# BatsResearch/menghini-neurips23-code

Hardware: AMD Instinct MI355X
Metric: images/sec CLIP ViT-B/16 encode+prompt-step (higher is better)
Workload: dtype f16

## Files before the change

### menghini-neurips23-code_amd/csrc/attention_split.hip

```cpp
#include <math.h>

#include "common.h"

__device__ __forceinline__ int vt_index_fwd_s(int key, int d) { return vt_index(key, ((d >> 2) & 3) * 16 + (d >> 4) * 4 + (d & 3)); }

__device__ __forceinline__ void split8(const f32x4 a, const f32x4 b, half8& hi, half8& lo) {
    half4 h0, l0, h1, l1;
    split_f16x4(a, h0, l0);
    split_f16x4(b, h1, l1);
    hi = (half8){h0[0], h0[1], h0[2], h0[3], h1[0], h1[1], h1[2], h1[3]};
    lo = (half8){l0[0], l0[1], l0[2], l0[3], l1[0], l1[1], l1[2], l1[3]};
}

template <int KVC, bool CAUSAL, int NW>
__global__ __launch_bounds__(NW * 64) void attn_fwd_split_kernel(const float* __restrict__ qkv, half_t* __restrict__ out, int S, int H) {
    constexpr int SP = KVC * 32;
    constexpr float LOG2E = 1.4426950408889634f;
    constexpr float INV = 1.0f / (float)GRIP_SPLIT_LO_SCALE;
    extern __shared__ __attribute__((aligned(16))) char smem[];
    half_t* Kh = (half_t*)smem;
    half_t* Kl = Kh + SP * 64;
    half_t* Vh = Kl + SP * 64;
    half_t* Vl = Vh + SP * 64;

    const int tid = threadIdx.x, lane = tid & 63, wave = tid >> 6;
    const int D = H * 64;
    const int b = blockIdx.x / H, h = blockIdx.x - b * H;
    const size_t ld = (size_t)3 * D;
    const float* base = qkv + (size_t)b * S * ld + h * 64;
    const int li = lane & 15, lg = lane >> 4;
    const int n_qt = (S + 15) >> 4;

    for (int idx = tid; idx < SP * 8; idx += NW * 64) {
        const int row = idx >> 3, chunk = idx & 7;
        f32x4 a = {0.f, 0.f, 0.f, 0.f}, c = {0.f, 0.f, 0.f, 0.f};
        if (row < S) {
            const f32x4* p = (const f32x4*)(base + (size_t)row * ld + D + chunk * 8);
            a = p[0];
            c = p[1];
        }
        half8 hi, lo;
        split8(a, c, hi, lo);
        const int o = row * 64 + ((chunk ^ (row & 7)) * 8);
        *(half8*)(Kh + o) = hi;
        *(half8*)(Kl + o) = lo;
    }
    for (int idx = tid; idx < ((SP / 2 + 31) / 32) * 256; idx += NW * 64) {
        const int lane_rp = idx & 31, chunk = ((idx >> 5) & 1) + 2 * ((idx >> 6) & 3), rblk = idx >> 8;
        const int r0 = 2 * (rblk * 32 + lane_rp);
        if (r0 >= SP) continue;
        f32x4 z = {0.f, 0.f, 0.f, 0.f};
        f32x4 a0 = z, a1 = z, b0 = z, b1 = z;
        if (r0 < S) { const f32x4* p = (const f32x4*)(base + (size_t)r0 * ld + 2 * D + chunk * 8); a0 = p[0]; a1 = p[1]; }
        if (r0 + 1 < S) { const f32x4* p = (const f32x4*)(base + (size_t)(r0 + 1) * ld + 2 * D + chunk * 8); b0 = p[0]; b1 = p[1]; }
        half8 h0, l0, h1, l1;
        split8(a0, a1, h0, l0);
        split8(b0, b1, h1, l1);
#pragma unroll
        for (int j = 0; j < 8; ++j) {
            const int o = vt_index_fwd_s(r0, chunk * 8 + j);
            *(half2v*)(Vh + o) = (half2v){h0[j], h1[j]};
            *(half2v*)(Vl + o) = (half2v){l0[j], l1[j]};
        }
    }
    __syncthreads();

    for (int qt = wave; qt < n_qt; qt += NW) {
        asm volatile("" ::: "memory");
        const int qrow = qt * 16 + li;
        const int qr = qrow < S ? qrow : S - 1;
        half8 qh[2], ql[2];
#pragma unroll
        for (int kk = 0; kk < 2; ++kk) {
            const f32x4* p = (const f32x4*)(base + (size_t)qr * ld + (kk * 4 + lg) * 8);
            split8(p[0] * 0.125f, p[1] * 0.125f, qh[kk], ql[kk]);
        }
        f32x4 sc[2 * KVC];
        float m = -INFINITY;
#pragma unroll
        for (int t = 0; t < 2 * KVC; ++t) {
            f32x4 acc = {0.f, 0.f, 0.f, 0.f}, cor = {0.f, 0.f, 0.f, 0.f};
#pragma unroll
            for (int kk = 0; kk < 2; ++kk) {
                const int o = (t * 16 + li) * 64 + (((kk * 4 + lg) ^ (lane & 7)) * 8);
                const half8 kh = *(const half8*)(Kh + o), kl = *(const half8*)(Kl + o);
                acc = __builtin_amdgcn_mfma_f32_16x16x32_f16(kh, qh[kk], acc, 0, 0, 0);
                cor = __builtin_amdgcn_mfma_f32_16x16x32_f16(kl, qh[kk], cor, 0, 0, 0);
                cor = __builtin_amdgcn_mfma_f32_16x16x32_f16(kh, ql[kk], cor, 0, 0, 0);
            }
            acc += cor * INV;
            if (CAUSAL || t >= 2 * (KVC - 1)) {
#pragma unroll
                for (int r = 0; r < 4; ++r) {
                    const int kv = t * 16 + lg * 4 + r;
                    if (kv >= S || (CAUSAL && kv > qrow)) acc[r] = -INFINITY;
                }
            }
            m = fmaxf(fmaxf(fmaxf(m, acc[0]), fmaxf(acc[1], acc[2])), acc[3]);
            sc[t] = acc;
        }
        m = fmaxf(m, __shfl_xor(m, 16));
        m = fmaxf(m, __shfl_xor(m, 32));
        const float m2 = m * LOG2E;
#pragma unroll
        for (int t = 0; t < 2 * KVC; ++t)
#pragma unroll
            for (int r = 0; r < 4; ++r) sc[t][r] = __builtin_amdgcn_exp2f(__builtin_fmaf(sc[t][r], LOG2E, -m2));

        const half8 ones = {1, 1, 1, 1, 1, 1, 1, 1};
        f32x4 sum_h = {0.f, 0.f, 0.f, 0.f}, sum_l = {0.f, 0.f, 0.f, 0.f};
        f32x4 o[4], oc[4];
#pragma unroll
        for (int nf = 0; nf < 4; ++nf) { o[nf] = (f32x4){0.f, 0.f, 0.f, 0.f}; oc[nf] = (f32x4){0.f, 0.f, 0.f, 0.f}; }
#pragma unroll
        for (int c = 0; c < KVC; ++c) {
            half8 ph, pl;
            split8(sc[2 * c], sc[2 * c + 1], ph, pl);
#pragma unroll
            for (int nf = 0; nf < 4; ++nf) {
                const int vo = (c * 4 + nf) * 512 + (lg * 16 + (li ^ lg)) * 8;
                const half8 vh = *(const half8*)(Vh + vo), vl = *(const half8*)(Vl + vo);
                o[nf] = __builtin_amdgcn_mfma_f32_16x16x32_f16(vh, ph, o[nf], 0, 0, 0);
                oc[nf] = __builtin_amdgcn_mfma_f32_16x16x32_f16(vl, ph, oc[nf], 0, 0, 0);
                oc[nf] = __builtin_amdgcn_mfma_f32_16x16x32_f16(vh, pl, oc[nf], 0, 0, 0);
            }
            sum_h = __builtin_amdgcn_mfma_f32_16x16x32_f16(ones, ph, sum_h, 0, 0, 0);
            sum_l = __builtin_amdgcn_mfma_f32_16x16x32_f16(ones, pl, sum_l, 0, 0, 0);
        }
        if (qrow < S) {
            const float inv = 1.0f / (sum_h[0] + sum_l[0] * INV);
            half_t* orow = out + (size_t)((size_t)b * S + qrow) * 2 * D;
            const int col = h * 64 + lg * 16;
            half_t* op = orow + (col >> 5) * 64 + (col & 31);
            half8 hi0, lo0, hi1, lo1;
            split8((o[0] + oc[0] * INV) * inv, (o[1] + oc[1] * INV) * inv, hi0, lo0);
            split8((o[2] + oc[2] * INV) * inv, (o[3] + oc[3] * INV) * inv, hi1, lo1);
            *(half8*)op = hi0;
            *(half8*)(op + 8) = hi1;
            *(half8*)(op + 32) = lo0;
            *(half8*)(op + 40) = lo1;
        }
    }
}

bool attention_split_supported(int S) { return S >= 1 && S <= 320; }

int launch_attention_fwd_split(const float* qkv, void* out, int B, int S, int H, int causal, hipStream_t s) {
    GRIP_REQUIRE(attention_split_supported(S) && B >= 1 && H >= 1, "attention_split: bad shape B=%d S=%d H=%d (S <= 320)", B, S, H);
    const int kvc = (S + 31) / 32;
    const size_t lds = (size_t)4 * kvc * 32 * 64 * sizeof(half_t);
#define GRIP_ATT_CASE(K)                                                                                                                     \
    case K: {                                                                                                                                \
        static bool configured = false;                                                                                                      \
        if (!configured) {                                                                                                                   \
            GRIP_CHECK_HIP(hipFuncSetAttribute((const void*)attn_fwd_split_kernel<K, false, (K >= 4 ? 8 : 4)>, hipFuncAttributeMaxDynamicSharedMemorySize, (int)lds)); \
            GRIP_CHECK_HIP(hipFuncSetAttribute((const void*)attn_fwd_split_kernel<K, true, (K >= 4 ? 8 : 4)>, hipFuncAttributeMaxDynamicSharedMemorySize, (int)lds));  \
            configured = true;                                                                                                               \
        }                                                                                                                                    \
        if (causal) hipLaunchKernelGGL((attn_fwd_split_kernel<K, true, (K >= 4 ? 8 : 4)>), dim3(B * H), dim3((K >= 4 ? 8 : 4) * 64), lds, s, qkv, (half_t*)out, S, H); \
        else hipLaunchKernelGGL((attn_fwd_split_kernel<K, false, (K >= 4 ? 8 : 4)>), dim3(B * H), dim3((K >= 4 ? 8 : 4) * 64), lds, s, qkv, (half_t*)out, S, H);       \
    } break;
    switch (kvc) {
        GRIP_ATT_CASE(1) GRIP_ATT_CASE(2) GRIP_ATT_CASE(3) GRIP_ATT_CASE(4) GRIP_ATT_CASE(5)
        GRIP_ATT_CASE(6) GRIP_ATT_CASE(7) GRIP_ATT_CASE(8) GRIP_ATT_CASE(9) GRIP_ATT_CASE(10)
        default: GRIP_REQUIRE(false, "attention_split: S = %d out of range", S);
    }
#undef GRIP_ATT_CASE
    GRIP_CHECK_HIP(hipGetLastError());
    return GRIP_OK;
}
```

Measured before the change: 21000.

## Make split attention persistent with register-prefetched K/V/Q for next head

Replaces the one-block-per-(batch,head) split-precision attention kernel with a persistent kernel for S up to 224 (KVC 1-7). Each block loops over items and prefetches the next item's K, V and Q from global memory into registers while computing scores and PV for the current one. This hides global load latency behind MFMA work and avoids relaunching blocks. Large S (KVC 8-10) moves to a flat kernel that always uses 8 waves. The persistent path raises register pressure, which could lower occupancy, and adds extra barriers per item.

```diff
diff --git a/menghini-neurips23-code_amd/csrc/attention_split.hip b/menghini-neurips23-code_amd/csrc/attention_split.hip
--- a/menghini-neurips23-code_amd/csrc/attention_split.hip
+++ b/menghini-neurips23-code_amd/csrc/attention_split.hip
@@ -12,11 +12,250 @@
     lo = (half8){l0[0], l0[1], l0[2], l0[3], l1[0], l1[1], l1[2], l1[3]};
 }
 
-template <int KVC, bool CAUSAL, int NW>
-__global__ __launch_bounds__(NW * 64) void attn_fwd_split_kernel(const float* __restrict__ qkv, half_t* __restrict__ out, int S, int H) {
-    constexpr int SP = KVC * 32;
+template <int KVC, bool CAUSAL>
+__device__ __forceinline__ void split_scores(const half_t* Kh, const half_t* Kl, const f32x4 (&qr)[2][2], int qrow, int S, int lane, f32x4 (&sc)[2 * KVC]) {
     constexpr float LOG2E = 1.4426950408889634f;
     constexpr float INV = 1.0f / (float)GRIP_SPLIT_LO_SCALE;
+    const int li = lane & 15, lg = lane >> 4;
+    half8 qh[2], ql[2];
+    int ko[2];
+#pragma unroll
+    for (int kk = 0; kk < 2; ++kk) {
+        split8(qr[kk][0] * 0.125f, qr[kk][1] * 0.125f, qh[kk], ql[kk]);
+        ko[kk] = li * 64 + (((kk * 4 + lg) ^ (lane & 7)) * 8);
+        asm volatile("" : "+v"(ko[kk]));
+    }
+    float m = -INFINITY;
+#pragma unroll
+    for (int t = 0; t < 2 * KVC; ++t) {
+        f32x4 acc = {0.f, 0.f, 0.f, 0.f}, cor = {0.f, 0.f, 0.f, 0.f};
+#pragma unroll
+        for (int kk = 0; kk < 2; ++kk) {
+            const int o = t * 16 * 64 + ko[kk];
+            const half8 kh = *(const half8*)(Kh + o), kl = *(const half8*)(Kl + o);
+            acc = __builtin_amdgcn_mfma_f32_16x16x32_f16(kh, qh[kk], acc, 0, 0, 0);
+            cor = __builtin_amdgcn_mfma_f32_16x16x32_f16(kl, qh[kk], cor, 0, 0, 0);
+            cor = __builtin_amdgcn_mfma_f32_16x16x32_f16(kh, ql[kk], cor, 0, 0, 0);
+        }
+        acc += cor * INV;
+        if (CAUSAL || t >= 2 * (KVC - 1)) {
+#pragma unroll
+            for (int r = 0; r < 4; ++r) {
+                const int kv = t * 16 + lg * 4 + r;
+                if (kv >= S || (CAUSAL && kv > qrow)) acc[r] = -INFINITY;
+            }
+        }
+        m = fmaxf(fmaxf(fmaxf(m, acc[0]), fmaxf(acc[1], acc[2])), acc[3]);
+        sc[t] = acc;
+    }
+    m = fmaxf(m, __shfl_xor(m, 16));
+    m = fmaxf(m, __shfl_xor(m, 32));
+    const float m2 = m * LOG2E;
+#pragma unroll
+    for (int t = 0; t < 2 * KVC; ++t)
+#pragma unroll
+        for (int r = 0; r < 4; ++r) sc[t][r] = __builtin_amdgcn_exp2f(__builtin_fmaf(sc[t][r], LOG2E, -m2));
+}
+
+template <int KVC>
+__device__ __forceinline__ void split_pv_store(const half_t* Vh, const half_t* Vl, const f32x4 (&sc)[2 * KVC], int qrow, int S, half_t* orow, int h, int lane) {
+    constexpr float INV = 1.0f / (float)GRIP_SPLIT_LO_SCALE;
+    const int li = lane & 15, lg = lane >> 4;
+    const half8 ones = {1, 1, 1, 1, 1, 1, 1, 1};
+    f32x4 sum_h = {0.f, 0.f, 0.f, 0.f}, sum_l = {0.f, 0.f, 0.f, 0.f};
+    f32x4 o[4], oc[4];
+    int vo0 = (lg * 16 + (li ^ lg)) * 8;
+    asm volatile("" : "+v"(vo0));
+#pragma unroll
+    for (int nf = 0; nf < 4; ++nf) { o[nf] = (f32x4){0.f, 0.f, 0.f, 0.f}; oc[nf] = (f32x4){0.f, 0.f, 0.f, 0.f}; }
+#pragma unroll
+    for (int c = 0; c < KVC; ++c) {
+        half8 ph, pl;
+        split8(sc[2 * c], sc[2 * c + 1], ph, pl);
+#pragma unroll
+        for (int nf = 0; nf < 4; ++nf) {
+            const int vo = (c * 4 + nf) * 512 + vo0;
+            const half8 vh = *(const half8*)(Vh + vo), vl = *(const half8*)(Vl + vo);
+            o[nf] = __builtin_amdgcn_mfma_f32_16x16x32_f16(vh, ph, o[nf], 0, 0, 0);
+            oc[nf] = __builtin_amdgcn_mfma_f32_16x16x32_f16(vl, ph, oc[nf], 0, 0, 0);
+            oc[nf] = __builtin_amdgcn_mfma_f32_16x16x32_f16(vh, pl, oc[nf], 0, 0, 0);
+        }
+        sum_h = __builtin_amdgcn_mfma_f32_16x16x32_f16(ones, ph, sum_h, 0, 0, 0);
+        sum_l = __builtin_amdgcn_mfma_f32_16x16x32_f16(ones, pl, sum_l, 0, 0, 0);
+    }
+    if (qrow < S) {
+        const float inv = 1.0f / (sum_h[0] + sum_l[0] * INV);
+        const int col = h * 64 + lg * 16;
+        half_t* op = orow + (col >> 5) * 64 + (col & 31);
+        half8 hi0, lo0, hi1, lo1;
+        split8((o[0] + oc[0] * INV) * inv, (o[1] + oc[1] * INV) * inv, hi0, lo0);
+        split8((o[2] + oc[2] * INV) * inv, (o[3] + oc[3] * INV) * inv, hi1, lo1);
+        *(half8*)op = hi0;
+        *(half8*)(op + 8) = hi1;
+        *(half8*)(op + 32) = lo0;
+        *(half8*)(op + 40) = lo1;
+    }
+}
+
+template <int KVC, bool CAUSAL, int NW>
+__global__ __launch_bounds__(NW * 64) void attn_fwd_split_kernel(const float* __restrict__ qkv, half_t* __restrict__ out, int S, int H, int n_items) {
+    constexpr int SP = KVC * 32;
+    constexpr int NQ = (2 * KVC + NW - 1) / NW;
+    constexpr int K_UNITS = SP * 8;
+    constexpr int NK = (K_UNITS + NW * 64 - 1) / (NW * 64);
+    constexpr int V_UNITS = ((SP / 2 + 31) / 32) * 256;
+    constexpr int NV = (V_UNITS + NW * 64 - 1) / (NW * 64);
+    extern __shared__ __attribute__((aligned(16))) char smem[];
+    half_t* Kh = (half_t*)smem;
+    half_t* Kl = Kh + SP * 64;
+    half_t* Vh = Kl + SP * 64;
+    half_t* Vl = Vh + SP * 64;
+
+    const int tid = threadIdx.x, lane = tid & 63;
+    const int wave = __builtin_amdgcn_readfirstlane(tid >> 6);
+    const int D = H * 64;
+    const size_t ld = (size_t)3 * D;
+    const int li = lane & 15, lg = lane >> 4;
+    const int n_qt = (S + 15) >> 4;
+
+    auto opaque_tid = [&]() {
+        int t = tid;
+        asm volatile("" : "+v"(t));
+        return t;
+    };
+    auto item_base = [&](int item) {
+        const int b = item / H, h = item - b * H;
+        return qkv + (size_t)b * S * ld + h * 64;
+    };
+    f32x4 kr[NK][2];
+    auto load_k = [&](const float* base) {
+        const int t0 = opaque_tid();
+#pragma unroll
+        for (int n = 0; n < NK; ++n) {
+            const int idx = t0 + n * NW * 64;
+            const int row = idx >> 3, chunk = idx & 7;
+            const f32x4* p = (const f32x4*)(base + (size_t)(row < S ? row : S - 1) * ld + D + chunk * 8);
+            kr[n][0] = p[0];
+            kr[n][1] = p[1];
+        }
+    };
+    auto store_k = [&]() {
+        const int t0 = opaque_tid();
+#pragma unroll
+        for (int n = 0; n < NK; ++n) {
+            const int idx = t0 + n * NW * 64;
+            const int row = idx >> 3, chunk = idx & 7;
+            if (idx < K_UNITS) {
+                const f32x4 z = {0.f, 0.f, 0.f, 0.f};
+                half8 hi, lo;
+                split8(row < S ? kr[n][0] : z, row < S ? kr[n][1] : z, hi, lo);
+                const int o = row * 64 + ((chunk ^ (row & 7)) * 8);
+                *(half8*)(Kh + o) = hi;
+                *(half8*)(Kl + o) = lo;
+            }
+        }
+    };
+    f32x4 vr[NV][4];
+    auto load_v = [&](const float* base) {
+        const int t0 = opaque_tid();
+#pragma unroll
+        for (int n = 0; n < NV; ++n) {
+            const int idx = t0 + n * NW * 64;
+            const int lane_rp = idx & 31, chunk = ((idx >> 5) & 1) + 2 * ((idx >> 6) & 3), rblk = idx >> 8;
+            const int r0 = 2 * (rblk * 32 + lane_rp);
+            const f32x4* p0 = (const f32x4*)(base + (size_t)(r0 < S ? r0 : S - 1) * ld + 2 * D + chunk * 8);
+            const f32x4* p1 = (const f32x4*)(base + (size_t)(r0 + 1 < S ? r0 + 1 : S - 1) * ld + 2 * D + chunk * 8);
+            vr[n][0] = p0[0]; vr[n][1] = p0[1];
+            vr[n][2] = p1[0]; vr[n][3] = p1[1];
+        }
+    };
+    auto store_v = [&]() {
+        const int t0 = opaque_tid();
+#pragma unroll
+        for (int n = 0; n < NV; ++n) {
+            const int idx = t0 + n * NW * 64;
+            const int lane_rp = idx & 31, chunk = ((idx >> 5) & 1) + 2 * ((idx >> 6) & 3), rblk = idx >> 8;
+            const int r0 = 2 * (rblk * 32 + lane_rp);
+            if (r0 < SP && idx < V_UNITS) {
+                const f32x4 z = {0.f, 0.f, 0.f, 0.f};
+                half8 h0, l0, h1, l1;
+                split8(r0 < S ? vr[n][0] : z, r0 < S ? vr[n][1] : z, h0, l0);
+                split8(r0 + 1 < S ? vr[n][2] : z, r0 + 1 < S ? vr[n][3] : z, h1, l1);
+#pragma unroll
+                for (int j = 0; j < 8; ++j) {
+                    const int o = vt_index_fwd_s(r0, chunk * 8 + j);
+                    *(half2v*)(Vh + o) = (half2v){h0[j], h1[j]};
+                    *(half2v*)(Vl + o) = (half2v){l0[j], l1[j]};
+                }
+            }
+        }
+    };
+    f32x4 qr[NQ][2][2];
+    auto load_q1 = [&](const float* base, int n) {
+        const int l0 = opaque_tid() & 63;
+        const int qrow = (wave + n * NW) * 16 + (l0 & 15);
+        const int qc = qrow < S ? qrow : S - 1;
+#pragma unroll
+        for (int kk = 0; kk < 2; ++kk) {
+            const f32x4* p = (const f32x4*)(base + (size_t)qc * ld + (kk * 4 + (l0 >> 4)) * 8);
+            qr[n][kk][0] = p[0];
+            qr[n][kk][1] = p[1];
+        }
+    };
+    auto barrier = [&]() {
+        asm volatile("s_waitcnt lgkmcnt(0)" ::: "memory");
+        __builtin_amdgcn_s_barrier();
+        asm volatile("" ::: "memory");
+    };
+
+    int item = blockIdx.x;
+    {
+        const float* base = item_base(item);
+        load_k(base);
+        load_v(base);
+#pragma unroll
+        for (int n = 0; n < NQ; ++n) load_q1(base, n);
+        store_k();
+    }
+    for (;;) {
+        barrier();
+        const int next = item + gridDim.x;
+        const bool has_next = next < n_items;
+        const float* nb = item_base(has_next ? next : item);
+        store_v();
+        const int b = item / H, h = item - b * H;
+        f32x4 sc[NQ][2 * KVC];
+#pragma unroll
+        for (int n = 0; n < NQ; ++n) {
+            const int qt = wave + n * NW;
+            if (qt < n_qt) {
+                asm volatile("" ::: "memory");
+                split_scores<KVC, CAUSAL>(Kh, Kl, qr[n], qt * 16 + li, S, lane, sc[n]);
+            }
+            if (n == 0) load_k(nb);
+        }
+        barrier();
+        if (has_next) store_k();
+#pragma unroll
+        for (int n = 0; n < NQ; ++n) {
+            const int qt = wave + n * NW;
+            if (qt < n_qt) {
+                asm volatile("" ::: "memory");
+                const int qrow = qt * 16 + li;
+                const int qs = qrow < S ? qrow : S - 1;
+                split_pv_store<KVC>(Vh, Vl, sc[n], qrow, S, out + ((size_t)b * S + qs) * 2 * D, h, lane);
+            }
+            load_q1(nb, n);
+            if (n == 0) load_v(nb);
+        }
+        if (!has_next) break;
+        item = next;
+    }
+}
+
+template <int KVC, bool CAUSAL, int NW>
+__global__ __launch_bounds__(NW * 64) void attn_fwd_split_flat_kernel(const float* __restrict__ qkv, half_t* __restrict__ out, int S, int H) {
+    constexpr int SP = KVC * 32;
     extern __shared__ __attribute__((aligned(16))) char smem[];
     half_t* Kh = (half_t*)smem;
     half_t* Kl = Kh + SP * 64;
@@ -68,104 +307,71 @@
     for (int qt = wave; qt < n_qt; qt += NW) {
         asm volatile("" ::: "memory");
         const int qrow = qt * 16 + li;
-        const int qr = qrow < S ? qrow : S - 1;
-        half8 qh[2], ql[2];
+        const int qs = qrow < S ? qrow : S - 1;
+        f32x4 qr[2][2];
 #pragma unroll
         for (int kk = 0; kk < 2; ++kk) {
-            const f32x4* p = (const f32x4*)(base + (size_t)qr * ld + (kk * 4 + lg) * 8);
-            split8(p[0] * 0.125f, p[1] * 0.125f, qh[kk], ql[kk]);
+            const f32x4* p = (const f32x4*)(base + (size_t)qs * ld + (kk * 4 + lg) * 8);
+            qr[kk][0] = p[0];
+            qr[kk][1] = p[1];
         }
         f32x4 sc[2 * KVC];
-        float m = -INFINITY;
-#pragma unroll
-        for (int t = 0; t < 2 * KVC; ++t) {
-            f32x4 acc = {0.f, 0.f, 0.f, 0.f}, cor = {0.f, 0.f, 0.f, 0.f};
-#pragma unroll
-            for (int kk = 0; kk < 2; ++kk) {
-                const int o = (t * 16 + li) * 64 + (((kk * 4 + lg) ^ (lane & 7)) * 8);
-                const half8 kh = *(const half8*)(Kh + o), kl = *(const half8*)(Kl + o);
-                acc = __builtin_amdgcn_mfma_f32_16x16x32_f16(kh, qh[kk], acc, 0, 0, 0);
-                cor = __builtin_amdgcn_mfma_f32_16x16x32_f16(kl, qh[kk], cor, 0, 0, 0);
-                cor = __builtin_amdgcn_mfma_f32_16x16x32_f16(kh, ql[kk], cor, 0, 0, 0);
-            }
-            acc += cor * INV;
-            if (CAUSAL || t >= 2 * (KVC - 1)) {
-#pragma unroll
-                for (int r = 0; r < 4; ++r) {
-                    const int kv = t * 16 + lg * 4 + r;
-                    if (kv >= S || (CAUSAL && kv > qrow)) acc[r] = -INFINITY;
-                }
-            }
-            m = fmaxf(fmaxf(fmaxf(m, acc[0]), fmaxf(acc[1], acc[2])), acc[3]);
-            sc[t] = acc;
-        }
-        m = fmaxf(m, __shfl_xor(m, 16));
-        m = fmaxf(m, __shfl_xor(m, 32));
-        const float m2 = m * LOG2E;
-#pragma unroll
-        for (int t = 0; t < 2 * KVC; ++t)
-#pragma unroll
-            for (int r = 0; r < 4; ++r) sc[t][r] = __builtin_amdgcn_exp2f(__builtin_fmaf(sc[t][r], LOG2E, -m2));
-
-        const half8 ones = {1, 1, 1, 1, 1, 1, 1, 1};
-        f32x4 sum_h = {0.f, 0.f, 0.f, 0.f}, sum_l = {0.f, 0.f, 0.f, 0.f};
-        f32x4 o[4], oc[4];
-#pragma unroll
-        for (int nf = 0; nf < 4; ++nf) { o[nf] = (f32x4){0.f, 0.f, 0.f, 0.f}; oc[nf] = (f32x4){0.f, 0.f, 0.f, 0.f}; }
-#pragma unroll
-        for (int c = 0; c < KVC; ++c) {
-            half8 ph, pl;
-            split8(sc[2 * c], sc[2 * c + 1], ph, pl);
-#pragma unroll
-            for (int nf = 0; nf < 4; ++nf) {
-                const int vo = (c * 4 + nf) * 512 + (lg * 16 + (li ^ lg)) * 8;
-                const half8 vh = *(const half8*)(Vh + vo), vl = *(const half8*)(Vl + vo);
-                o[nf] = __builtin_amdgcn_mfma_f32_16x16x32_f16(vh, ph, o[nf], 0, 0, 0);
-                oc[nf] = __builtin_amdgcn_mfma_f32_16x16x32_f16(vl, ph, oc[nf], 0, 0, 0);
-                oc[nf] = __builtin_amdgcn_mfma_f32_16x16x32_f16(vh, pl, oc[nf], 0, 0, 0);
-            }
-            sum_h = __builtin_amdgcn_mfma_f32_16x16x32_f16(ones, ph, sum_h, 0, 0, 0);
-            sum_l = __builtin_amdgcn_mfma_f32_16x16x32_f16(ones, pl, sum_l, 0, 0, 0);
-        }
-        if (qrow < S) {
-            const float inv = 1.0f / (sum_h[0] + sum_l[0] * INV);
-            half_t* orow = out + (size_t)((size_t)b * S + qrow) * 2 * D;
-            const int col = h * 64 + lg * 16;
-            half_t* op = orow + (col >> 5) * 64 + (col & 31);
-            half8 hi0, lo0, hi1, lo1;
-            split8((o[0] + oc[0] * INV) * inv, (o[1] + oc[1] * INV) * inv, hi0, lo0);
-            split8((o[2] + oc[2] * INV) * inv, (o[3] + oc[3] * INV) * inv, hi1, lo1);
-            *(half8*)op = hi0;
-            *(half8*)(op + 8) = hi1;
-            *(half8*)(op + 32) = lo0;
-            *(half8*)(op + 40) = lo1;
-        }
+        split_scores<KVC, CAUSAL>(Kh, Kl, qr, qrow, S, lane, sc);
+        split_pv_store<KVC>(Vh, Vl, sc, qrow, S, out + ((size_t)b * S + qs) * 2 * D, h, lane);
     }
 }
 
 bool attention_split_supported(int S) { return S >= 1 && S <= 320; }
+
+template <int KVC, bool CAUSAL>
+static int launch_split_persistent(const float* qkv, half_t* out, int B, int S, int H, hipStream_t s) {
+    constexpr int NW = KVC >= 4 ? 8 : 4;
+    constexpr size_t lds = (size_t)4 * KVC * 32 * 64 * sizeof(half_t);
+    static int resident = 0, per_cu_s = 0;
+    if (!resident) {
+        GRIP_CHECK_HIP(hipFuncSetAttribute((const void*)attn_fwd_split_kernel<KVC, CAUSAL, NW>, hipFuncAttributeMaxDynamicSharedMemorySize, (int)lds));
+        int dev = 0, n_cu = 0, per_cu = 0;
+        GRIP_CHECK_HIP(hipGetDevice(&dev));
+        GRIP_CHECK_HIP(hipDeviceGetAttribute(&n_cu, hipDeviceAttributeMultiprocessorCount, dev));
+        GRIP_CHECK_HIP(hipOccupancyMaxActiveBlocksPerMultiprocessor(&per_cu, attn_fwd_split_kernel<KVC, CAUSAL, NW>, NW * 64, lds));
+        GRIP_REQUIRE(per_cu >= 1, "attention_split: the persistent kernel does not fit a CU (KVC %d)", KVC);
+        resident = n_cu * per_cu;
+        per_cu_s = per_cu;
+    }
+    const int n_items = B * H;
+    const int width = (grip_cu_budget() > 0 && grip_cu_budget() * per_cu_s < resident) ? grip_cu_budget() * per_cu_s : resident;
+    const int grid = n_items < width ? n_items : width;
+    hipLaunchKernelGGL((attn_fwd_split_kernel<KVC, CAUSAL, NW>), dim3(grid), dim3(NW * 64), lds, s, qkv, out, S, H, n_items);
+    GRIP_CHECK_HIP(hipGetLastError());
+    return GRIP_OK;
+}
+
+template <int KVC, bool CAUSAL>
+static int launch_split_flat(const float* qkv, half_t* out, int B, int S, int H, hipStream_t s) {
+    constexpr int NW = 8;
+    constexpr size_t lds = (size_t)4 * KVC * 32 * 64 * sizeof(half_t);
+    static bool configured = false;
+    if (!configured) {
+        GRIP_CHECK_HIP(hipFuncSetAttribute((const void*)attn_fwd_split_flat_kernel<KVC, CAUSAL, NW>, hipFuncAttributeMaxDynamicSharedMemorySize, (int)lds));
+        configured = true;
+    }
+    hipLaunchKernelGGL((attn_fwd_split_flat_kernel<KVC, CAUSAL, NW>), dim3(B * H), dim3(NW * 64), lds, s, qkv, out, S, H);
+    GRIP_CHECK_HIP(hipGetLastError());
+    return GRIP_OK;
+}
 
 int launch_attention_fwd_split(const float* qkv, void* out, int B, int S, int H, int causal, hipStream_t s) {
     GRIP_REQUIRE(attention_split_supported(S) && B >= 1 && H >= 1, "attention_split: bad shape B=%d S=%d H=%d (S <= 320)", B, S, H);
     const int kvc = (S + 31) / 32;
-    const size_t lds = (size_t)4 * kvc * 32 * 64 * sizeof(half_t);
-#define GRIP_ATT_CASE(K)                                                                                                                     \
-    case K: {                                                                                                                                \
-        static bool configured = false;                                                                                                      \
-        if (!configured) {                                                                                                                   \
-            GRIP_CHECK_HIP(hipFuncSetAttribute((const void*)attn_fwd_split_kernel<K, false, (K >= 4 ? 8 : 4)>, hipFuncAttributeMaxDynamicSharedMemorySize, (int)lds)); \
-            GRIP_CHECK_HIP(hipFuncSetAttribute((const void*)attn_fwd_split_kernel<K, true, (K >= 4 ? 8 : 4)>, hipFuncAttributeMaxDynamicSharedMemorySize, (int)lds));  \
-            configured = true;                                                                                                               \
-        }                                                                                                                                    \
-        if (causal) hipLaunchKernelGGL((attn_fwd_split_kernel<K, true, (K >= 4 ? 8 : 4)>), dim3(B * H), dim3((K >= 4 ? 8 : 4) * 64), lds, s, qkv, (half_t*)out, S, H); \
-        else hipLaunchKernelGGL((attn_fwd_split_kernel<K, false, (K >= 4 ? 8 : 4)>), dim3(B * H), dim3((K >= 4 ? 8 : 4) * 64), lds, s, qkv, (half_t*)out, S, H);       \
-    } break;
+#define GRIP_ATT_CASE(K, F) \
+    case K: return causal ? F<K, true>(qkv, (half_t*)out, B, S, H, s) : F<K, false>(qkv, (half_t*)out, B, S, H, s);
     switch (kvc) {
-        GRIP_ATT_CASE(1) GRIP_ATT_CASE(2) GRIP_ATT_CASE(3) GRIP_ATT_CASE(4) GRIP_ATT_CASE(5)
-        GRIP_ATT_CASE(6) GRIP_ATT_CASE(7) GRIP_ATT_CASE(8) GRIP_ATT_CASE(9) GRIP_ATT_CASE(10)
+        GRIP_ATT_CASE(1, launch_split_persistent) GRIP_ATT_CASE(2, launch_split_persistent) GRIP_ATT_CASE(3, launch_split_persistent)
+        GRIP_ATT_CASE(4, launch_split_persistent) GRIP_ATT_CASE(5, launch_split_persistent) GRIP_ATT_CASE(6, launch_split_persistent)
+        GRIP_ATT_CASE(7, launch_split_persistent)
+        GRIP_ATT_CASE(8, launch_split_flat) GRIP_ATT_CASE(9, launch_split_flat) GRIP_ATT_CASE(10, launch_split_flat)
         default: GRIP_REQUIRE(false, "attention_split: S = %d out of range", S);
     }
 #undef GRIP_ATT_CASE
-    GRIP_CHECK_HIP(hipGetLastError());
     return GRIP_OK;
 }
```

New measurement: 21050 (median of 2 runs). About the same (+0.2%).
